# xitorch/xitorch

Hardware: AMD Instinct MI355X
Metric: eigpairs/sec of symeig(davidson) + Lanczos-role matvec GB/s (roofline.achieved), batch=64 N=16384 (higher is better)
Workload: dtype f64

## Files before the change

### xitorch_amd/csrc/xk_basis.hip

```cpp
#include "xk_common.h"

namespace xk {

template <typename T, int P>
__global__ __launch_bounds__(256) void lincomb_kernel(
    const T* __restrict__ V, const T* __restrict__ C, T* __restrict__ Out,
    int k, int N, long ldv, long sV, long sC, long sCa, long sCc, long ldo, long sO,
    T alpha, T beta, int col_tiles) {
  typedef typename Vec16<T>::type VT;
  constexpr int VN = Vec16<T>::n;
  const int b = blockIdx.x / col_tiles;
  const int ct = blockIdx.x - b * col_tiles;
  const int j = (ct * 256 + threadIdx.x) * VN;
  if (j >= N) return;
  const T* Vb = V + (long)b * sV + j;
  const T* Cb = C + (long)b * sC;
  VT acc[P];
#pragma unroll
  for (int c = 0; c < P; ++c)
#pragma unroll
    for (int v = 0; v < VN; ++v) acc[c][v] = T(0);
  int a = 0;
  for (; a + 8 <= k; a += 8) {
    VT v[8];
#pragma unroll
    for (int u = 0; u < 8; ++u) v[u] = *reinterpret_cast<const VT*>(Vb + (long)(a + u) * ldv);
#pragma unroll
    for (int c = 0; c < P; ++c) {
      T cc[8];
#pragma unroll
      for (int u = 0; u < 8; ++u) cc[u] = Cb[(long)(a + u) * sCa + c * sCc];
#pragma unroll
      for (int u = 0; u < 8; ++u)
#pragma unroll
        for (int e = 0; e < VN; ++e) acc[c][e] += cc[u] * v[u][e];
    }
  }
  for (; a + 4 <= k; a += 4) {
    VT v0 = *reinterpret_cast<const VT*>(Vb + (long)(a + 0) * ldv);
    VT v1 = *reinterpret_cast<const VT*>(Vb + (long)(a + 1) * ldv);
    VT v2 = *reinterpret_cast<const VT*>(Vb + (long)(a + 2) * ldv);
    VT v3 = *reinterpret_cast<const VT*>(Vb + (long)(a + 3) * ldv);
#pragma unroll
    for (int c = 0; c < P; ++c) {
      const T c0 = Cb[(long)(a + 0) * sCa + c * sCc], c1 = Cb[(long)(a + 1) * sCa + c * sCc];
      const T c2 = Cb[(long)(a + 2) * sCa + c * sCc], c3 = Cb[(long)(a + 3) * sCa + c * sCc];
#pragma unroll
      for (int v = 0; v < VN; ++v) {
        acc[c][v] += c0 * v0[v];
        acc[c][v] += c1 * v1[v];
        acc[c][v] += c2 * v2[v];
        acc[c][v] += c3 * v3[v];
      }
    }
  }
  for (; a < k; ++a) {
    VT v0 = *reinterpret_cast<const VT*>(Vb + (long)a * ldv);
#pragma unroll
    for (int c = 0; c < P; ++c) {
      const T c0 = Cb[(long)a * sCa + c * sCc];
#pragma unroll
      for (int v = 0; v < VN; ++v) acc[c][v] += c0 * v0[v];
    }
  }
  T* Ob = Out + (long)b * sO + j;
#pragma unroll
  for (int c = 0; c < P; ++c) {
    VT o;
    if (beta != T(0)) {
      o = *reinterpret_cast<const VT*>(Ob + (long)c * ldo);
#pragma unroll
      for (int v = 0; v < VN; ++v) o[v] = beta * o[v] + alpha * acc[c][v];
    } else {
#pragma unroll
      for (int v = 0; v < VN; ++v) o[v] = alpha * acc[c][v];
    }
    *reinterpret_cast<VT*>(Ob + (long)c * ldo) = o;
  }
}

template <typename T, int P>
__global__ __launch_bounds__(256) void ritz_residual_kernel(
    const T* __restrict__ V, const T* __restrict__ AV, const T* __restrict__ Y,
    const T* __restrict__ lam, T* __restrict__ X, T* __restrict__ Tn, T* __restrict__ rmax,
    int k, int N, long ldv, long sV, long ldav, long sAV, long sY, long sYa, long sYc, long sLam,
    long ldx, long sX, long ldt, long sT, int col_tiles) {
  typedef typename Vec16<T>::type VT;
  constexpr int VN = Vec16<T>::n;
  __shared__ T red[4];
  const int b = blockIdx.x / col_tiles;
  const int ct = blockIdx.x - b * col_tiles;
  const int j = (ct * 256 + threadIdx.x) * VN;
  const bool active = j < N;
  T local_max = T(0);
  if (active) {
    const T* Vb = V + (long)b * sV + j;
    const T* AVb = AV + (long)b * sAV + j;
    const T* Yb = Y + (long)b * sY;
    VT ax[P], xx[P];
#pragma unroll
    for (int c = 0; c < P; ++c)
#pragma unroll
      for (int v = 0; v < VN; ++v) { ax[c][v] = T(0); xx[c][v] = T(0); }
    int a = 0;
    for (; a + 4 <= k; a += 4) {
      VT v[4], w[4];
#pragma unroll
      for (int u = 0; u < 4; ++u) {
        v[u] = *reinterpret_cast<const VT*>(Vb + (long)(a + u) * ldv);
        w[u] = *reinterpret_cast<const VT*>(AVb + (long)(a + u) * ldav);
      }
#pragma unroll
      for (int c = 0; c < P; ++c) {
        T yy[4];
#pragma unroll
        for (int u = 0; u < 4; ++u) yy[u] = Yb[(long)(a + u) * sYa + c * sYc];
#pragma unroll
        for (int u = 0; u < 4; ++u)
#pragma unroll
          for (int e = 0; e < VN; ++e) {
            xx[c][e] += yy[u] * v[u][e];
            ax[c][e] += yy[u] * w[u][e];
          }
      }
    }
    for (; a + 2 <= k; a += 2) {
      VT v0 = *reinterpret_cast<const VT*>(Vb + (long)a * ldv);
      VT v1 = *reinterpret_cast<const VT*>(Vb + (long)(a + 1) * ldv);
      VT w0 = *reinterpret_cast<const VT*>(AVb + (long)a * ldav);
      VT w1 = *reinterpret_cast<const VT*>(AVb + (long)(a + 1) * ldav);
#pragma unroll
      for (int c = 0; c < P; ++c) {
        const T y0 = Yb[(long)a * sYa + c * sYc], y1 = Yb[(long)(a + 1) * sYa + c * sYc];
#pragma unroll
        for (int v = 0; v < VN; ++v) {
          xx[c][v] += y0 * v0[v];
          xx[c][v] += y1 * v1[v];
          ax[c][v] += y0 * w0[v];
          ax[c][v] += y1 * w1[v];
        }
      }
    }
    for (; a < k; ++a) {
      VT v0 = *reinterpret_cast<const VT*>(Vb + (long)a * ldv);
      VT w0 = *reinterpret_cast<const VT*>(AVb + (long)a * ldav);
#pragma unroll
      for (int c = 0; c < P; ++c) {
        const T y0 = Yb[(long)a * sYa + c * sYc];
#pragma unroll
        for (int v = 0; v < VN; ++v) { xx[c][v] += y0 * v0[v]; ax[c][v] += y0 * w0[v]; }
      }
    }
#pragma unroll
    for (int c = 0; c < P; ++c) {
      const T l = lam[(long)b * sLam + c];
      VT t;
#pragma unroll
      for (int v = 0; v < VN; ++v) {
        const T r = ax[c][v] - l * xx[c][v];
        t[v] = -r;
        T ar = r < T(0) ? -r : r;
        ar = ar != ar ? T(INFINITY) : ar;
        local_max = ar > local_max ? ar : local_max;
      }
      *reinterpret_cast<VT*>(X + (long)b * sX + (long)c * ldx + j) = xx[c];
      *reinterpret_cast<VT*>(Tn + (long)b * sT + (long)c * ldt + j) = t;
    }
  }
  local_max = wave_max(local_max);
  if ((threadIdx.x & 63) == 0) red[threadIdx.x >> 6] = local_max;
  __syncthreads();
  if (threadIdx.x == 0) {
    T m = red[0];
    m = red[1] > m ? red[1] : m;
    m = red[2] > m ? red[2] : m;
    m = red[3] > m ? red[3] : m;
    atomic_max_nonneg(rmax + b, m);
  }
}

template <typename T>
__global__ __launch_bounds__(64) void panel_chol_kernel(const T* __restrict__ G, T* __restrict__ W, int* __restrict__ info,
                                                        int B, int P, long ldg, long sG, long sW) {
  __shared__ T R[32][33];
  __shared__ T C[32][33];
  const int b = blockIdx.x;
  const int j = threadIdx.x;
  if (b >= B) return;
  const T* Gb = G + (long)b * sG;
  const bool own = j < P;
  int bad = 0;
  for (int i = 0; i < P; ++i) {
    T s = T(0);
    if (own && j >= i) {
      s = T(0.5) * (Gb[(long)i * ldg + j] + Gb[(long)j * ldg + i]);
      for (int m = 0; m < i; ++m) s -= R[m][i] * R[m][j];
      if (j == i) {
        if (!(s > T(0))) { bad = i + 1; s = T(1); }
        R[i][i] = sqrt(s);
      }
    }
    __builtin_amdgcn_fence(__ATOMIC_RELEASE, "wavefront");
    __builtin_amdgcn_wave_barrier();
    __builtin_amdgcn_fence(__ATOMIC_ACQUIRE, "wavefront");
    if (own && j > i) R[i][j] = s / R[i][i];
    if (own && j < i) R[i][j] = T(0);
    __builtin_amdgcn_fence(__ATOMIC_RELEASE, "wavefront");
    __builtin_amdgcn_wave_barrier();
    __builtin_amdgcn_fence(__ATOMIC_ACQUIRE, "wavefront");
  }
  T* Wb = W + (long)b * sW;
  if (own) {
    const int c = j;
    for (int i = P - 1; i >= 0; --i) {
      T s = (i == c) ? T(1) : T(0);
      for (int m = i + 1; m <= c; ++m) s -= R[i][m] * C[m][c];
      C[i][c] = (i <= c) ? s / R[i][i] : T(0);
    }
    for (int i = 0; i < P; ++i) Wb[(long)i * P + c] = C[i][c];
  }
  const unsigned long long flagged = __ballot(bad != 0);
  if (flagged && j == (int)(__ffsll((long long)flagged) - 1)) info[b] = bad;
}

template <typename T>
__global__ __launch_bounds__(256) void panel_transform_kernel(
    T* __restrict__ Tp, const T* __restrict__ W, int P, int N, long ldt, long sT, long sW, int col_tiles) {
  typedef typename Vec16<T>::type VT;
  constexpr int VN = Vec16<T>::n;
  const int b = blockIdx.x / col_tiles;
  const int ct = blockIdx.x - b * col_tiles;
  const int j = (ct * 256 + threadIdx.x) * VN;
  if (j >= N) return;
  T* Tb = Tp + (long)b * sT + j;
  const T* Wb = W + (long)b * sW;
  for (int c = P - 1; c >= 0; --c) {
    VT acc;
#pragma unroll
    for (int v = 0; v < VN; ++v) acc[v] = T(0);
    for (int a = 0; a <= c; ++a) {
      const T w = Wb[(long)a * P + c];
      VT t = *reinterpret_cast<const VT*>(Tb + (long)a * ldt);
#pragma unroll
      for (int v = 0; v < VN; ++v) acc[v] += w * t[v];
    }
    *reinterpret_cast<VT*>(Tb + (long)c * ldt) = acc;
  }
}

template <typename T>
static bool vec_ok(int N, long ld, long s, const void* p) {
  constexpr int VN = Vec16<T>::n;
  const long npad = ((long)N + VN - 1) / VN * VN;
  return (ld % VN == 0) && (ld >= npad || ld == 0) && (s % VN == 0) && (((uintptr_t)p & 15) == 0);
}

template <typename T>
static int lincomb(const T* V, const T* C, T* Out, int B, int k, int N, int P, long ldv, long sV,
                   long sC, long sCa, long sCc, long ldo, long sO, T alpha, T beta, hipStream_t st) {
  constexpr int VN = Vec16<T>::n;
  if (!vec_ok<T>(N, ldv, sV, V) || !vec_ok<T>(N, ldo, sO, Out)) return XK_ERR_UNSUPPORTED;
  const int ct = (N + 256 * VN - 1) / (256 * VN);
  int c0 = 0;
  while (c0 < P) {
    const int pc = (P - c0) >= 8 ? 8 : (P - c0);
    const T* Cc = C + (long)c0 * sCc;
    T* Oc = Out + (long)c0 * ldo;
    switch (pc) {
#define XK_CASE(PP)                                                                                   \
  case PP:                                                                                            \
    hipLaunchKernelGGL((lincomb_kernel<T, PP>), dim3((unsigned)((long)B * ct)), dim3(256), 0, st, V, \
                       Cc, Oc, k, N, ldv, sV, sC, sCa, sCc, ldo, sO, alpha, beta, ct);                \
    break;
      XK_CASE(1) XK_CASE(2) XK_CASE(3) XK_CASE(4) XK_CASE(5) XK_CASE(6) XK_CASE(7) XK_CASE(8)
#undef XK_CASE
    }
    XK_LAUNCH_CHECK();
    c0 += pc;
  }
  return XK_OK;
}

template <typename T>
static int ritz_residual(const T* V, const T* AV, const T* Y, const T* lam, T* X, T* Tn, T* rmax, int B,
                         int k, int N, int P, long ldv, long sV, long ldav, long sAV, long sY, long sYa,
                         long sYc, long sLam, long ldx, long sX, long ldt, long sT, hipStream_t st) {
  constexpr int VN = Vec16<T>::n;
  if (!vec_ok<T>(N, ldv, sV, V) || !vec_ok<T>(N, ldav, sAV, AV) || !vec_ok<T>(N, ldx, sX, X) ||
      !vec_ok<T>(N, ldt, sT, Tn))
    return XK_ERR_UNSUPPORTED;
  const int ct = (N + 256 * VN - 1) / (256 * VN);
  int c0 = 0;
  while (c0 < P) {
    const int pc = (P - c0) >= 8 ? 8 : (P - c0);
    switch (pc) {
#define XK_CASE(PP)                                                                                    \
  case PP:                                                                                             \
    hipLaunchKernelGGL((ritz_residual_kernel<T, PP>), dim3((unsigned)((long)B * ct)), dim3(256), 0,   \
                       st, V, AV, Y + (long)c0 * sYc, lam + c0, X + (long)c0 * ldx, Tn + (long)c0 * ldt, \
                       rmax, k, N, ldv, sV, ldav, sAV, sY, sYa, sYc, sLam, ldx, sX, ldt, sT, ct);       \
    break;
      XK_CASE(1) XK_CASE(2) XK_CASE(3) XK_CASE(4) XK_CASE(5) XK_CASE(6) XK_CASE(7) XK_CASE(8)
#undef XK_CASE
    }
    XK_LAUNCH_CHECK();
    c0 += pc;
  }
  return XK_OK;
}


template <typename T>
__global__ __launch_bounds__(256) void diag_precond_kernel(T* __restrict__ Tn, const T* __restrict__ d,
                                                            const T* __restrict__ m, const T* __restrict__ lam,
                                                            int N, int P, long ldt, long sT, long sD, long sM,
                                                            long sLam, T floor_, long total) {
  const long idx = (long)blockIdx.x * 256 + threadIdx.x;
  if (idx >= total) return;
  const long per_b = (long)P * N;
  const long b = idx / per_b;
  const long rem = idx - b * per_b;
  const int c = (int)(rem / N);
  const int n = (int)(rem - (long)c * N);
  const T mm = m ? m[b * sM + n] : T(1);
  T den = d[b * sD + n] - lam[b * sLam + c] * mm;
  if (fabs(den) < floor_) den = den < T(0) ? -floor_ : floor_;
  T* t = Tn + b * sT + (long)c * ldt + n;
  *t = *t / den;
}

template <typename T>
__global__ __launch_bounds__(64) void group_status_kernel(const T* __restrict__ rmax, const int* __restrict__ info,
                                                          const int* __restrict__ flag, T* __restrict__ orth,
                                                          double* __restrict__ status, int B) {
  const int lane = threadIdx.x;
  double m = 0.0, om_ = 0.0;
  int nan = 0, i1 = 0, i2 = 0;
  bool first = true;
  for (int b = lane; b < B; b += 64) {
    const double v = (double)rmax[b];
    nan |= (v != v);
    m = first ? v : (v > m ? v : m);
    const int a = info[b];
    i1 = first ? a : (a > i1 ? a : i1);
    if (flag) {
      const int f = flag[b];
      i2 = first ? f : (f > i2 ? f : i2);
    }
    if (orth) {
      const double ov = (double)orth[b];
      orth[b] = T(0);
      om_ = (ov != ov) ? __builtin_inf() : (ov > om_ ? ov : om_);
    }
    first = false;
  }
  double mm = first ? -__builtin_inf() : m;
  int a1 = first ? -2147483647 - 1 : i1, a2 = first ? -2147483647 - 1 : i2;
#pragma unroll
  for (int sft = 32; sft >= 1; sft >>= 1) {
    const double om = __shfl_xor(mm, sft, 64), oo = __shfl_xor(om_, sft, 64);
    const int o1 = __shfl_xor(a1, sft, 64), o2 = __shfl_xor(a2, sft, 64), on = __shfl_xor(nan, sft, 64);
    mm = om > mm ? om : mm;
    om_ = oo > om_ ? oo : om_;
    a1 = o1 > a1 ? o1 : a1;
    a2 = o2 > a2 ? o2 : a2;
    nan |= on;
  }
  if (lane == 0) {
    status[0] = nan ? __builtin_nan("") : mm;
    status[1] = (double)a1;
    status[2] = flag ? (double)a2 : 0.0;
    if (orth) status[4] = om_;
  }
// ... 76 lines not shown
```

### xitorch_amd/csrc/xk_common.h

```cpp
#pragma once
#include <hip/hip_runtime.h>
#include <stdint.h>

#define XK_WAVE 64

#define XK_OK 0
#define XK_ERR_ARG (-1)
#define XK_ERR_UNSUPPORTED (-2)

#define XK_LAUNCH_CHECK()                       \
  do {                                          \
    hipError_t e__ = hipGetLastError();         \
    if (e__ != hipSuccess) return (int)e__;     \
  } while (0)

namespace xk {

typedef double d2 __attribute__((ext_vector_type(2)));
typedef float f4 __attribute__((ext_vector_type(4)));

template <typename T> struct Vec16;
template <> struct Vec16<double> { typedef d2 type; static constexpr int n = 2; };
template <> struct Vec16<float> { typedef f4 type; static constexpr int n = 4; };

template <typename V>
__device__ __forceinline__ V ld_stream(const V* p) {
  return __builtin_nontemporal_load(p);
}

__device__ __forceinline__ double shfl_xor_t(double v, int mask) { return __shfl_xor(v, mask, 64); }
__device__ __forceinline__ float shfl_xor_t(float v, int mask) { return __shfl_xor(v, mask, 64); }

template <int CTRL, int ROW_MASK>
__device__ __forceinline__ double dpp_shift_or_zero(double v) {
  const int lo = __builtin_amdgcn_update_dpp(0, __double2loint(v), CTRL, ROW_MASK, 0xf, true);
  const int hi = __builtin_amdgcn_update_dpp(0, __double2hiint(v), CTRL, ROW_MASK, 0xf, true);
  return __hiloint2double(hi, lo);
}
template <int CTRL, int ROW_MASK>
__device__ __forceinline__ float dpp_shift_or_zero(float v) {
  return __int_as_float(__builtin_amdgcn_update_dpp(0, __float_as_int(v), CTRL, ROW_MASK, 0xf, true));
}
template <int MASK> struct PartnerCtrl;
template <> struct PartnerCtrl<8> { static constexpr int ctrl = 0x128; };
template <> struct PartnerCtrl<4> { static constexpr int ctrl = 0x141; };
template <> struct PartnerCtrl<2> { static constexpr int ctrl = 0x4e; };
template <> struct PartnerCtrl<1> { static constexpr int ctrl = 0xb1; };
template <int MASK>
__device__ __forceinline__ double lane_partner(double v) {
  const int lo = __builtin_amdgcn_update_dpp(0, __double2loint(v), PartnerCtrl<MASK>::ctrl, 0xf, 0xf, false);
  const int hi = __builtin_amdgcn_update_dpp(0, __double2hiint(v), PartnerCtrl<MASK>::ctrl, 0xf, 0xf, false);
  return __hiloint2double(hi, lo);
}
template <int MASK>
__device__ __forceinline__ float lane_partner(float v) {
  return __int_as_float(__builtin_amdgcn_update_dpp(0, __float_as_int(v), PartnerCtrl<MASK>::ctrl, 0xf, 0xf, false));
}
template <typename T>
__device__ __forceinline__ T lane_partner_rt(T v, int mask) {
  switch (mask) {
    case 8: return lane_partner<8>(v);
    case 4: return lane_partner<4>(v);
    case 2: return lane_partner<2>(v);
    case 1: return lane_partner<1>(v);
    default: return shfl_xor_t(v, mask);
  }
}
__device__ __forceinline__ double readlane63(double v) {
  const int lo = __builtin_amdgcn_readlane(__double2loint(v), 63);
  const int hi = __builtin_amdgcn_readlane(__double2hiint(v), 63);
  return __hiloint2double(hi, lo);
}
__device__ __forceinline__ float readlane63(float v) {
  return __int_as_float(__builtin_amdgcn_readlane(__float_as_int(v), 63));
}
template <typename T>
__device__ __forceinline__ T wave_sum_dpp(T v) {
  v += dpp_shift_or_zero<0x111, 0xf>(v);
  v += dpp_shift_or_zero<0x112, 0xf>(v);
  v += dpp_shift_or_zero<0x114, 0xf>(v);
  v += dpp_shift_or_zero<0x118, 0xf>(v);
  v += dpp_shift_or_zero<0x142, 0xa>(v);
  v += dpp_shift_or_zero<0x143, 0xc>(v);
  return readlane63(v);
}

template <typename T>
__device__ __forceinline__ T wave_max(T v) {
#pragma unroll
  for (int m = 32; m >= 1; m >>= 1) {
    T o = shfl_xor_t(v, m);
    v = o > v ? o : v;
  }
  return v;
}

template <int NV> struct HalvingStages {
  static constexpr int value = (NV % 2 == 0 && NV > 1) ? 1 + HalvingStages<NV / 2>::value : 0;
};
template <> struct HalvingStages<1> { static constexpr int value = 0; };
template <> struct HalvingStages<0> { static constexpr int value = 0; };

__device__ __forceinline__ double swap_add32(double a, double b) {
  auto lo = __builtin_amdgcn_permlane32_swap((unsigned)__double2loint(a), (unsigned)__double2loint(b), false, false);
  auto hi = __builtin_amdgcn_permlane32_swap((unsigned)__double2hiint(a), (unsigned)__double2hiint(b), false, false);
  return __hiloint2double((int)hi[0], (int)lo[0]) + __hiloint2double((int)hi[1], (int)lo[1]);
}
__device__ __forceinline__ float swap_add32(float a, float b) {
  auto r = __builtin_amdgcn_permlane32_swap(__float_as_uint(a), __float_as_uint(b), false, false);
  return __uint_as_float(r[0]) + __uint_as_float(r[1]);
// ... 92 lines not shown
```

### xitorch_amd/csrc/xk_symm.hip

```cpp
#include "xk_common.h"

namespace xk {

constexpr int SYMM_TRH = 1024;
constexpr long SYMM_SMALL_LAUNCH = 2200;
constexpr int SYMM_NU = 2;
constexpr int SYMM_R = 8;
constexpr long SYMM_QUEUE_ELEMS = 16;

typedef __amdgpu_buffer_rsrc_t TileRsrc;
typedef unsigned int u4 __attribute__((ext_vector_type(4)));
constexpr unsigned SYMM_OOR = 0x7ffffff0u;

#ifndef XK_SYMM_AUX
#define XK_SYMM_AUX 2
#endif
template <typename VT>
__device__ __forceinline__ VT ld_tile(const TileRsrc rsrc, unsigned lane_off, unsigned s_off) {
  const u4 raw = __builtin_amdgcn_raw_buffer_load_b128(rsrc, (int)lane_off, (int)s_off, XK_SYMM_AUX);
  return __builtin_bit_cast(VT, raw);
}

template <typename T>
__device__ __forceinline__ TileRsrc make_tile_rsrc(const T* tile_base, long bytes) {
// ... 344 lines not shown
  int j = 0;
#pragma unroll 1
  for (;;) {
#pragma unroll 1
    for (; q < NW; ++q) {
      int rb, re, c0, dg;
      if (symm_range<T, TRH, NW>(run, j, q, rb, re, c0, dg)) {
        SymmNext after = symm_next_range<T, TRH, NW>(run, j, q);
        if (after.row < 0) { after.row = run.row0; after.last = run.row0; after.col0 = N; }
        symm_rows<T, P, false>(a, tile, Xb, ldab, ldx, rb, re, run.row0, col0, N, jj, after, acc_col, xJ,
                               rowacc, lane);
      }
      __syncthreads();
    }
    T* cp = colP + (((long)b * NT + I) * P) * (long)N;
#pragma unroll
    for (int u = 0; u < NU; ++u)
      if (jj[u] < N) {
        if (flags & 1) {
#pragma unroll
          for (int c = 0; c < P; ++c) __builtin_nontemporal_store(acc_col[u][c], reinterpret_cast<VT*>(cp + (long)c * N + jj[u]));
        } else {
#pragma unroll
          for (int c = 0; c < P; ++c) *reinterpret_cast<VT*>(cp + (long)c * N + jj[u]) = acc_col[u][c];
        }
      }
    if (++j >= run.ntile) break;
    q = 0;
    col0 = (run.J0 + j) * SLAB;
    symm_tile_setup<T, P>(Xb, (int)ldx, col0, N, lanecol, jj, acc_col, xJ);
  }
  {
    const int k3 = (NW - 1) ^ run.sig;
    const int fb = run.row0 + k3 * SYMM_QR;
    int fe = fb + SYMM_QR;
    fe = fe < run.tile_end ? fe : run.tile_end;
    const int nr = fe - fb;
    T* rp = rowP + (((long)b * NSL + slot) * P) * (long)N;
    for (int idx = lane; idx < nr * P; idx += 64) {
      const int c = idx / nr, lr = idx - c * nr;
      const T v = rowacc[(fb - run.row0 + lr) * P + c];
      if (flags & 1) __builtin_nontemporal_store(v, &rp[(long)c * N + fb + lr]);
      else rp[(long)c * N + fb + lr] = v;
    }
  }
  if (!PERSIST) break;
  __syncthreads();
  item = __builtin_amdgcn_readfirstlane(s_next[par]);
  par ^= 1;
  }
}

template <typename T, int PP, bool PERS>
static int symm_launch_wide8(dim3 grid, size_t lds, hipStream_t st, const T* A, const T* Xc, T* rowP, T* colP,
                             int nruns, int N, long lda, long sA, long ldx, long sX, int NS, int NT, int NSL, int L,
                             int fl, unsigned* queue, int nitems) {
  if constexpr (sizeof(T) == 8) {
    auto kfn = dense_symm_tiles<T, PP, 2048, PERS, 8>;
    if (lds > 65536) {
      hipError_t ae = hipFuncSetAttribute(reinterpret_cast<const void*>(kfn),
                                          hipFuncAttributeMaxDynamicSharedMemorySize, (int)lds);
      if (ae != hipSuccess) return (int)ae;
    }
    hipLaunchKernelGGL(kfn, grid, dim3(512), lds, st, A, Xc, rowP, colP, nruns, N, lda, sA, ldx, sX, NS, NT, NSL, L,
                       fl, queue, nitems);
    return XK_OK;
  } else {
    return XK_ERR_UNSUPPORTED;
  }
}

static int symm_device_cus() {
  static int cus[64] = {0};
  int dev = 0;
  if (hipGetDevice(&dev) != hipSuccess || dev < 0 || dev >= 64) return 256;
  if (cus[dev] == 0) {
    int n = 0;
    if (hipDeviceGetAttribute(&n, hipDeviceAttributeMultiprocessorCount, dev) != hipSuccess || n <= 0) n = 256;
    cus[dev] = n;
  }
  return cus[dev];
}

template <typename T>
__global__ __launch_bounds__(256) void symm_fold(const T* __restrict__ rowP, const T* __restrict__ colP,
                                                  T* __restrict__ Y, int N, int P, int NS, int NT, int NSL, int L,
                                                  int slab, long ldy, long sY, long total, int flags, int trh) {
  const long idx = (long)blockIdx.x * 256 + threadIdx.x;
  if (idx >= total) return;
  const long per_b = (long)P * N;
  const long b = idx / per_b;
  const long rem = idx - b * per_b;
  const int c = (int)(rem / N);
  const int n = (int)(rem - (long)c * N);
  const int It = n / trh;
  const int jmin = (It * trh) / slab;
  const int nslot = (NS - jmin + L - 1) / L;
  T s = T(0);
  const int Imax = ((n / slab) * slab + slab - 1) / trh;
  if (flags & 2) {
    for (int r = 0; r < nslot; ++r) s += __builtin_nontemporal_load(&rowP[(((long)b * NSL + r) * P + c) * (long)N + n]);
    for (int I = 0; I <= Imax && I < NT; ++I)
      s += __builtin_nontemporal_load(&colP[(((long)b * NT + I) * P + c) * (long)N + n]);
  } else {
    for (int r = 0; r < nslot; ++r) s += rowP[(((long)b * NSL + r) * P + c) * (long)N + n];
    for (int I = 0; I <= Imax && I < NT; ++I) s += colP[(((long)b * NT + I) * P + c) * (long)N + n];
  }
  Y[b * sY + (long)c * ldy + n] = s;
}

}

extern "C" {


long xk_dense_symm_workspace_elems(int B, int N, int P, int elem_size) {
  const int vn = 16 / elem_size;
  const long slab = 256L * vn * xk::SYMM_NU;
  const long NS = (N + slab - 1) / slab, NT = (N + 511) / 512;
  const long pc = P > 6 ? 6 : P;
  return (long)B * (NS + NT) * pc * N + xk::SYMM_QUEUE_ELEMS;
}

#define XK_DEFINE_SYMM(SUF, T)                                                                              \
  static int symm_launch_##SUF(const T* A, const T* X, T* Y, T* ws, long ws_elems, int B, int N, int P,     \
                               long lda, long sA, long ldx, long sX, long ldy, long sY, int opts,           \
                               void* stream, int phase) {                                                   \
    if (B < 0 || N < 0 || P < 0 || opts < 0 || opts > 0x0fffffff) return XK_ERR_ARG;                        \
    if (B == 0 || N == 0 || P == 0) return XK_OK;                                                           \
    if (phase != 0 && P > 6) return XK_ERR_UNSUPPORTED;            \
    constexpr int VN = xk::Vec16<T>::n;                                                                     \
                       \
    const bool wide8 = sizeof(T) == 8 && (opts & 32) != 0;                                                  \
    const int NWV = wide8 ? 8 : 4;                                                                          \
    const int SLAB = NWV * 64 * VN * xk::SYMM_NU;                                                           \
    if ((N % VN) || (lda % VN) || (sA % VN) || (ldx % VN) || (sX % VN) || ((uintptr_t)A & 15) ||             \
        ((uintptr_t)X & 15) || ((uintptr_t)ws & 15))                                                        \
      return XK_ERR_UNSUPPORTED;                                                                            \
    if ((long)(wide8 ? 2048 : xk::SYMM_TRH) * lda * (long)sizeof(T) > 0x7fffffe0L) return XK_ERR_UNSUPPORTED; \
    hipStream_t st = (hipStream_t)stream;                                                                   \
    const int L = ((opts >> 8) & 0xff) ? ((opts >> 8) & 0xff) : 1, fl = 3 & ~opts;                          \
    const bool persist = (opts & 16) != 0;                                                                  \
    int nslots = (opts >> 16) & 0xfff;                                                                      \
    if (persist && nslots == 0) nslots = 2 * xk::symm_device_cus();                                         \
    if (persist && wide8) nslots = (nslots + 1) / 2;               \
    if (persist && (nslots <= 0 || ws_elems < xk::SYMM_QUEUE_ELEMS)) return XK_ERR_ARG;                     \
    unsigned* queue = persist ? reinterpret_cast<unsigned*>(ws + (ws_elems - xk::SYMM_QUEUE_ELEMS)) : nullptr; \
    if (persist) ws_elems -= xk::SYMM_QUEUE_ELEMS;                                                          \
    if (L > 64) return XK_ERR_ARG;                                                                          \
    const int NS = (N + SLAB - 1) / SLAB;                                                                   \
    const int NSL = (NS + L - 1) / L;                                                                       \
         \
    int trh = xk::SYMM_TRH;                                                                                 \
    {                                                                                                       \
      const int nt1 = (N + xk::SYMM_TRH - 1) / xk::SYMM_TRH;                                                \
      long nr1 = 0;                                                                                         \
      for (int I = 0; I < nt1; ++I) nr1 += (NS - (I * xk::SYMM_TRH) / SLAB + L - 1) / L;                    \
      if (sizeof(T) == 8 && (long)B * nr1 < xk::SYMM_SMALL_LAUNCH) trh = 512;                               \
      if (sizeof(T) == 8 && (opts & 4)) trh = 512;                                                          \
      if (opts & 8) trh = xk::SYMM_TRH;                                                                     \
      if (wide8) trh = 2048;                                                                                \
    }                                                                                                       \
    const int NT = (N + trh - 1) / trh;                                                                     \
    int nruns = 0;                                                                                          \
    for (int I = 0; I < NT; ++I) nruns += (NS - (I * trh) / SLAB + L - 1) / L;                              \
    int c0 = 0;                                                                                             \
    while (c0 < P) {                                                                                        \
      const int pc = (P - c0) >= 6 ? 6 : (P - c0);                                                          \
      const long nrow = (long)B * NSL * pc * N, ncol = (long)B * NT * pc * N;                               \
      if (ws_elems < nrow + ncol) return XK_ERR_ARG;                                                        \
      T* rowP = ws;                                                                                         \
      T* colP = ws + nrow;                                                                                  \
      const size_t lds = (size_t)trh * pc * sizeof(T);                                                      \
      const long nitems_l = (long)B * nruns;                                                                \
      if (nitems_l > 0x7fffffffL) return XK_ERR_UNSUPPORTED;                                                \
      const int nitems = (int)nitems_l;                                                                     \
      const dim3 grid((unsigned)(persist ? (nitems < nslots ? nitems : nslots) : nitems));                  \
      const T* Xc = X + (long)c0 * ldx;                                                                     \
      if (phase != 2) {                                                                                     \
        if (persist) {                                                                                      \
          hipError_t me = hipMemsetAsync(queue, 0, 64, st);                                                 \
          if (me != hipSuccess) return (int)me;                                                             \
        }                                                                                                   \
        switch (pc) {                                                                                       \
          XK_SYMM_CASE(1) XK_SYMM_CASE(2) XK_SYMM_CASE(3) XK_SYMM_CASE(4) XK_SYMM_CASE(5) XK_SYMM_CASE(6)   \
        }                                                                                                   \
        XK_LAUNCH_CHECK();                                                                                  \
      }                                                                                                     \
      if (phase != 1) {                                                                                     \
        const long total = (long)B * pc * N;                                                                \
        hipLaunchKernelGGL((xk::symm_fold<T>), dim3((unsigned)((total + 255) / 256)), dim3(256), 0, st,     \
                           rowP, colP, Y + (long)c0 * ldy, N, pc, NS, NT, NSL, L, SLAB, ldy, sY, total,     \
                           fl, trh);                                                                        \
        XK_LAUNCH_CHECK();                                                                                  \
      }                                                                                                     \
      c0 += pc;                                                                                             \
    }                                                                                                       \
    return XK_OK;                                                                                           \
  }                                                                                                         \
  int xk_dense_symm_##SUF(const T* A, const T* X, T* Y, T* ws, long ws_elems, int B, int N, int P, long lda, \
                          long sA, long ldx, long sX, long ldy, long sY, int opts, void* stream) {          \
    return symm_launch_##SUF(A, X, Y, ws, ws_elems, B, N, P, lda, sA, ldx, sX, ldy, sY, opts, stream, 0);   \
  }                                                                                                         \
  int xk_dense_symm_tiles_##SUF(const T* A, const T* X, T* ws, long ws_elems, int B, int N, int P,          \
                                long lda, long sA, long ldx, long sX, int opts, void* stream) {             \
    return symm_launch_##SUF(A, X, (T*)nullptr, ws, ws_elems, B, N, P, lda, sA, ldx, sX, 0, 0, opts,        \
                             stream, 1);                                                                    \
  }                                                                                                         \
  int xk_dense_symm_fold_##SUF(T* Y, const T* ws, long ws_elems, int B, int N, int P, long ldy, long sY,    \
                               int opts, void* stream) {                                                    \
                                         \
    return symm_launch_##SUF((const T*)ws, (const T*)ws, Y, (T*)ws, ws_elems, B, N, P, N, 0, N, 0, ldy, sY, \
                             opts, stream, 2);                                                              \
  }

#define XK_SYMM_LAUNCH(PP, RR, PERS)                                                                      \
  hipLaunchKernelGGL((xk::dense_symm_tiles<TT, PP, RR, PERS, 4>), grid, dim3(256), lds, st, A, Xc, rowP, colP, \
                     nruns, N, lda, sA, ldx, sX, NS, NT, NSL, L, fl, queue, nitems)
#define XK_SYMM_WIDE8(PP, PERS)                                                                           \
  do {                                                                                                    \
    const int wrc = xk::symm_launch_wide8<TT, PP, PERS>(grid, lds, st, A, Xc, rowP, colP, nruns, N, lda, sA, ldx, \
                                                        sX, NS, NT, NSL, L, fl, queue, nitems);           \
    if (wrc != XK_OK) return wrc;                                                                         \
  } while (0)
#define XK_SYMM_CASE(PP)                                                                                  \
  case PP:                                                                                                \
    if (wide8) {                                                                                          \
      if (persist) XK_SYMM_WIDE8(PP, true); else XK_SYMM_WIDE8(PP, false);                                \
    } else if (trh == 512) {                                                                              \
      if (persist) XK_SYMM_LAUNCH(PP, 512, true); else XK_SYMM_LAUNCH(PP, 512, false);                    \
    } else {                                                                                              \
      if (persist) XK_SYMM_LAUNCH(PP, 1024, true); else XK_SYMM_LAUNCH(PP, 1024, false);                  \
    }                                                                                                     \
    break;

#define TT double
XK_DEFINE_SYMM(f64, double)
#undef TT
#define TT float
XK_DEFINE_SYMM(f32, float)
#undef TT

}
```

### xitorch_amd/linalg/native_eig.py

```python
import os
import torch
from xitorch_amd import kernels as K
from xitorch_amd._capi import NativeLibraryError
from xitorch_amd._util import bcast_shape
from xitorch_amd.linalg._panel import PanelOperator, pad_len
from xitorch_amd.dist import allreduce_max_

__all__ = ["davidson", "exacteig", "take_eigpairs", "tallqr_extend", "native_partial_eigh"]

_PRELAUNCH = True
CHAIN_CUS = "all"
K3G_MAX_K = [1536, 1024]
K3P_MIN_K = int(os.environ.get("XITORCH_K3P_MIN_K", "80"))


def take_eigpairs(evals, evecs, neig, mode):
    if mode == "lowest":
        return evals[..., :neig], evecs[..., :neig]
    return evals[..., -neig:], evecs[..., -neig:]


def _pad(n, dtype):
    return pad_len(n)

# ... 427 lines not shown
GUARD_MAX_REDO = 3


def davidson(A, neig, mode, M=None, max_niter=1000, nguess=None, v_init="randn", max_addition=None,
             min_eps=1e-6, verbose=False, V0=None, orth_passes="auto", process_group=None, trace=None,
             rng_device="cpu", small_eigh="native", overlap="auto", precond=None, reserve_cus="auto", restart=None,
             groups="auto", chain="calls", basis_capacity=None, **unused):
    kw = dict(M=M, max_niter=max_niter, nguess=nguess, v_init=v_init, max_addition=max_addition, min_eps=min_eps,
              verbose=verbose, V0=V0, process_group=process_group, trace=trace, rng_device=rng_device,
              small_eigh=small_eigh, overlap=overlap, precond=precond, reserve_cus=reserve_cus, restart=restart,
              groups=groups, chain=chain, basis_capacity=basis_capacity, **unused)
    try:
        return _davidson(A, neig, mode, orth_passes=orth_passes, **kw)
    except _GuardFailure as err:
        if isinstance(orth_passes, int) and orth_passes >= 3:
            raise RuntimeError("xitorch_amd davidson: %s" % err)
        first = dict(trace) if trace is not None else None
        try:
            res = _davidson(A, neig, mode, orth_passes=3, **kw)
        except _GuardFailure as err2:
            raise RuntimeError("xitorch_amd davidson: %s (also with three orthogonalisation passes)" % err2)
        if trace is not None:
            trace["orth_rerun"] = {"reason": str(err), "first_run": {k: first.get(k) for k in ("niter", "orth_redo")}}
        return res


class _GuardPolicy:

    def __init__(self, dtype, k_start):
        self.good, self.bad = GUARD_GOOD[dtype], GUARD_BAD[dtype]
        self.k_good = k_start
        self.history, self.redo = [], []
        self._restarts = 0

    def seen(self, guard, nrestart):
        self.history.append(guard)
        if nrestart != self._restarts:
            self._restarts, self.k_good = nrestart, None

    def void(self, chol_flag, guard):
        return chol_flag != 0 or guard > self.bad

    def roll_back(self, chol_flag, guard, k_rr, niter, trace):
        if self.k_good is None or self.k_good >= k_rr or len(self.redo) >= GUARD_MAX_REDO:
            if chol_flag != 0 and not self.redo:
                raise RuntimeError("xitorch_amd davidson: the panel Gram matrix is not positive definite "
                                   "(linearly dependent guess/residual vectors)")
            if trace is not None:
                trace.update(niter=niter, orth_redo=self.redo, orth_guard_history=self.history)
            raise _GuardFailure("the Ritz block lost its orthonormality (max|X^T M X - I| = %.2e at iteration %d, "
                                "basis of %d vectors) and no earlier basis is left to return to" % (guard, niter, k_rr))
        self.redo.append({"iter": niter, "guard": guard, "chol_flag": chol_flag, "k_from": k_rr, "k_to": self.k_good,
                          "passes": 2 + len(self.redo)})
        return self.k_good, 2 + len(self.redo) - 1

    def passed(self, guard, k_rr):
        if guard <= self.good:
            self.k_good = k_rr
            return True
        return False


class _Plan:
    __slots__ = ("two", "ngrp", "reserve_cus", "spans", "ops", "streams", "k1_streams", "k1_sched", "distributed")


def _plan_groups(A, whole, M, B, N, p, dtype, device, precond, overlap, groups, reserve_cus, k1_streams_opt,
                 reserve_schedule, process_group):
    plan = _Plan()
    nA = 1
    for d in A.shape[:-2]:
        nA *= d
    can_two = M is None and whole.kind == "dense" and not whole.flip and nA == B and B >= 2 \
        and not (precond is not None and not isinstance(precond, (str, torch.Tensor)))
    big = B * N * N * (8 if dtype == torch.float64 else 4) >= 2 ** 33
    two = can_two and (overlap is True or (overlap == "auto" and big))
    ngrp = 2
    if two:
        if groups == "auto":
            ngrp = 2
        else:
            ngrp = max(2, min(int(groups), B))
    reserve_auto = reserve_cus == "auto"
    if reserve_cus == "auto":
        wide_symm = whole.kind == "dense" and whole.symm and dtype == torch.float32 and \
            K.SYMM_WIDE_MIN_P <= p <= K.SYMM_WIDE_MAX_P and N >= K.SYMM_WIDE_MIN_N and N % 64 == 0
        reserve_cus = 32 if wide_symm else 64
        if can_two and K.K1S_OPTS is None and whole.kind == "dense" and whole.symm and whole.symm_narrow and p <= 6 \
                and (k1_streams_opt == "auto" or bool(k1_streams_opt)):
            total_cus = torch.cuda.get_device_properties(device).multi_processor_count
            if K.k1s_auto_opts(B // ngrp, N, dtype, max(1, total_cus - 32), pipelined=True) & K.K1S_PERSIST:
                reserve_cus = 32
    grp_streams, k1_streams, k1_sched = None, [None], None
    if two:
        try:
            chain_reserved = CHAIN_CUS == "reserved" or (CHAIN_CUS == "auto" and wide_symm and bool(K.K1SW_OPTS & 8))
            if chain_reserved and reserve_cus > 0:
                grp_streams = [K.masked_stream(device, reserve_cus, slot=1 + g, only_reserved=True) for g in range(ngrp)]
            else:
                grp_streams = [K.masked_stream(device, 0, slot=1 + g) for g in range(ngrp)]
            k1_stream = K.masked_stream(device, reserve_cus)
            k1_streams = [k1_stream] * ngrp
            if k1_streams_opt == "auto":
                k1o = K.K1S_OPTS if K.K1S_OPTS is not None else \
                    K.k1s_auto_opts(B // ngrp, N, dtype, K.stream_cus(k1_stream), pipelined=True)
                split_k1 = bool(k1o & K.K1S_PERSIST) and whole.kind == "dense" and whole.symm \
                    and whole.symm_narrow and p <= 6
            else:
                split_k1 = bool(k1_streams_opt)
            if k1_streams_opt == "auto" and not split_k1 and whole.kind == "dense" and whole.symm and \
                    dtype == torch.float32 and K.SYMM_WIDE_MIN_P <= p <= K.SYMM_WIDE_MAX_P and \
                    N >= K.SYMM_WIDE_MIN_N and N % 64 == 0:
                split_k1 = bool(K._k1sw_opts(k1_stream, B // ngrp, N, pipelined=True) & K.K1SW_PERSIST)
            if split_k1:
                k1_streams = [K.masked_stream(device, reserve_cus, slot=64 + g) for g in range(ngrp)]
                sched = reserve_schedule
                if sched == "auto":
                    sched = [(0, 32), (132, 64)] if (reserve_auto and reserve_cus == 32) else None
                if sched:
                    k1_sched = [(int(kf), [K.masked_stream(device, int(reserve_cus if cu is None else cu), slot=64 + g)
                                           for g in range(ngrp)]) for (kf, cu) in sched]
        except NativeLibraryError as err:
            import warnings
            warnings.warn("xitorch_amd davidson: CU-masked streams unavailable (%s); running one batch group" % err)
            two = False
    distributed = process_group is not None and torch.distributed.get_world_size(process_group) > 1
    if distributed:
        g_local = ngrp if two else 1
        g_all = torch.tensor([-float(g_local)], dtype=torch.float64, device=device)
        torch.distributed.all_reduce(g_all, op=torch.distributed.ReduceOp.MAX, group=process_group)
        g_common = int(round(-g_all.item()))
        if g_common < g_local:
            if g_common <= 1:
                two = False
            else:
                ngrp = g_common
                grp_streams, k1_streams = grp_streams[:ngrp], k1_streams[:ngrp]
                k1_sched = [(kf, sts[:ngrp]) for (kf, sts) in k1_sched] if k1_sched is not None else None
    if two:
        cuts = [(B * g) // ngrp for g in range(ngrp + 1)]
        spans = [(cuts[g], cuts[g + 1]) for g in range(ngrp)]
        ops = [_PanelOperator(_sub_operator(A, B, N, b0, b1), [b1 - b0], b1 - b0, N) for (b0, b1) in spans]
        cur = torch.cuda.current_stream()
        streams = grp_streams
        for st in streams + list(set(k1_streams)) + [t for (_, sts) in (k1_sched or []) for t in sts]:
            st.wait_stream(cur)
    else:
        spans, ops, streams, k1_streams, k1_sched = [(0, B)], [whole], [torch.cuda.current_stream()], [None], None
    plan.two, plan.ngrp, plan.reserve_cus, plan.spans, plan.ops, plan.streams = two, ngrp, reserve_cus, spans, ops, streams
    plan.k1_streams, plan.k1_sched, plan.distributed = k1_streams, k1_sched, distributed
    return plan


def _preconditioner(precond, whole, M, bdims, B, N, dtype, device):
    if precond is None:
        return None
    from xitorch_amd.linop import LinearOperator as _LinOp
    if isinstance(precond, str):
        if precond.lower() not in ("diag", "jacobi", "davidson"):
            raise RuntimeError("Unknown davidson preconditioner: %s" % precond)
        dA = whole.diagonal()
        dM = _PanelOperator(M, bdims, B, N).diagonal() if M is not None else None
        return ("diag", dA, dM)
    if isinstance(precond, torch.Tensor):
        if precond.shape[-1] != N:
            raise RuntimeError("precond diagonal must have shape (*batch, %d), got %s" % (N, tuple(precond.shape)))
        dA = precond.to(device=device, dtype=dtype).expand(*bdims, N).reshape(B, N).contiguous()
        dM = _PanelOperator(M, bdims, B, N).diagonal() if M is not None else None
        return ("diag", dA, dM)
# ... 317 lines not shown
```

Measured before the change: 1827.

## Use buffer-resource ring-buffered row loads in lincomb, ritz residual and symm fold

Rewrites the basis lincomb and Ritz-residual kernels to keep a register ring of in-flight row loads (depth 16 and 8), issued as raw buffer loads with scalar offsets and guarded out-of-range so the memory pipeline stays full. symm_fold is vectorized to 16-byte accesses per thread with the same ring prefetch. A Python fix hoists wide_symm out of the auto branch so it is defined when reserve_cus is explicit. This aims to hide memory latency in bandwidth-bound streaming kernels, at the cost of higher register pressure and new span limits that fall back to unsupported for large strides.

```diff
diff --git a/xitorch_amd/csrc/xk_basis.hip b/xitorch_amd/csrc/xk_basis.hip
--- a/xitorch_amd/csrc/xk_basis.hip
+++ b/xitorch_amd/csrc/xk_basis.hip
@@ -1,6 +1,12 @@
 #include "xk_common.h"
 
 namespace xk {
+
+constexpr int LINCOMB_RING = 16;
+constexpr int RITZ_RING = 8;
+#ifndef XK_BASIS_AUX
+#define XK_BASIS_AUX 0
+#endif
 
 template <typename T, int P>
 __global__ __launch_bounds__(256) void lincomb_kernel(
@@ -9,58 +15,56 @@
     T alpha, T beta, int col_tiles) {
   typedef typename Vec16<T>::type VT;
   constexpr int VN = Vec16<T>::n;
+  constexpr int D = LINCOMB_RING;
   const int b = blockIdx.x / col_tiles;
   const int ct = blockIdx.x - b * col_tiles;
   const int j = (ct * 256 + threadIdx.x) * VN;
   if (j >= N) return;
-  const T* Vb = V + (long)b * sV + j;
+  const T* Vb = V + (long)b * sV;
   const T* Cb = C + (long)b * sC;
+  const unsigned loff = (unsigned)j * (unsigned)sizeof(T);
+  const unsigned ldvb = (unsigned)(ldv * (long)sizeof(T));
   VT acc[P];
 #pragma unroll
   for (int c = 0; c < P; ++c)
 #pragma unroll
     for (int v = 0; v < VN; ++v) acc[c][v] = T(0);
+  VT ring[D];
+  RowRsrc rs = make_row_rsrc(Vb);
+#pragma unroll
+  for (int u = 0; u < D; ++u) ring[u] = ld_row<VT, XK_BASIS_AUX>(rs, u < k ? loff : ROW_OOR, (unsigned)u * ldvb);
   int a = 0;
-  for (; a + 8 <= k; a += 8) {
-    VT v[8];
-#pragma unroll
-    for (int u = 0; u < 8; ++u) v[u] = *reinterpret_cast<const VT*>(Vb + (long)(a + u) * ldv);
-#pragma unroll
-    for (int c = 0; c < P; ++c) {
-      T cc[8];
-#pragma unroll
-      for (int u = 0; u < 8; ++u) cc[u] = Cb[(long)(a + u) * sCa + c * sCc];
-#pragma unroll
-      for (int u = 0; u < 8; ++u)
-#pragma unroll
-        for (int e = 0; e < VN; ++e) acc[c][e] += cc[u] * v[u][e];
-    }
-  }
-  for (; a + 4 <= k; a += 4) {
-    VT v0 = *reinterpret_cast<const VT*>(Vb + (long)(a + 0) * ldv);
-    VT v1 = *reinterpret_cast<const VT*>(Vb + (long)(a + 1) * ldv);
-    VT v2 = *reinterpret_cast<const VT*>(Vb + (long)(a + 2) * ldv);
-    VT v3 = *reinterpret_cast<const VT*>(Vb + (long)(a + 3) * ldv);
-#pragma unroll
-    for (int c = 0; c < P; ++c) {
-      const T c0 = Cb[(long)(a + 0) * sCa + c * sCc], c1 = Cb[(long)(a + 1) * sCa + c * sCc];
-      const T c2 = Cb[(long)(a + 2) * sCa + c * sCc], c3 = Cb[(long)(a + 3) * sCa + c * sCc];
-#pragma unroll
-      for (int v = 0; v < VN; ++v) {
-        acc[c][v] += c0 * v0[v];
-        acc[c][v] += c1 * v1[v];
-        acc[c][v] += c2 * v2[v];
-        acc[c][v] += c3 * v3[v];
-      }
-    }
-  }
-  for (; a < k; ++a) {
-    VT v0 = *reinterpret_cast<const VT*>(Vb + (long)a * ldv);
-#pragma unroll
-    for (int c = 0; c < P; ++c) {
-      const T c0 = Cb[(long)a * sCa + c * sCc];
-#pragma unroll
-      for (int v = 0; v < VN; ++v) acc[c][v] += c0 * v0[v];
+  for (; a + D <= k; a += D) {
+#pragma unroll
+    for (int h = 0; h < D; h += 4) {
+      T cc[4][P];
+#pragma unroll
+      for (int u = 0; u < 4; ++u)
+#pragma unroll
+        for (int c = 0; c < P; ++c) cc[u][c] = Cb[(long)(a + h + u) * sCa + c * sCc];
+#pragma unroll
+      for (int u = 0; u < 4; ++u) {
+        const VT v = ring[h + u];
+#pragma unroll
+        for (int c = 0; c < P; ++c)
+#pragma unroll
+          for (int e = 0; e < VN; ++e) acc[c][e] += cc[u][c] * v[e];
+        ring[h + u] = ld_row<VT, XK_BASIS_AUX>(rs, a + D + h + u < k ? loff : ROW_OOR, (unsigned)(D + h + u) * ldvb);
+        __builtin_amdgcn_sched_barrier(0);
+      }
+    }
+    rs = make_row_rsrc(Vb + (long)(a + D) * ldv);
+  }
+#pragma unroll
+  for (int u = 0; u < D - 1; ++u) {
+    if (a + u < k) {
+      const VT v = ring[u];
+#pragma unroll
+      for (int c = 0; c < P; ++c) {
+        const T c0 = Cb[(long)(a + u) * sCa + c * sCc];
+#pragma unroll
+        for (int e = 0; e < VN; ++e) acc[c][e] += c0 * v[e];
+      }
     }
   }
   T* Ob = Out + (long)b * sO + j;
@@ -87,6 +91,7 @@
     long ldx, long sX, long ldt, long sT, int col_tiles) {
   typedef typename Vec16<T>::type VT;
   constexpr int VN = Vec16<T>::n;
+  constexpr int D = RITZ_RING;
   __shared__ T red[4];
   const int b = blockIdx.x / col_tiles;
   const int ct = blockIdx.x - b * col_tiles;
@@ -94,61 +99,61 @@
   const bool active = j < N;
   T local_max = T(0);
   if (active) {
-    const T* Vb = V + (long)b * sV + j;
-    const T* AVb = AV + (long)b * sAV + j;
+    const T* Vb = V + (long)b * sV;
+    const T* AVb = AV + (long)b * sAV;
     const T* Yb = Y + (long)b * sY;
+    const unsigned loff = (unsigned)j * (unsigned)sizeof(T);
+    const unsigned ldvb = (unsigned)(ldv * (long)sizeof(T)), ldavb = (unsigned)(ldav * (long)sizeof(T));
     VT ax[P], xx[P];
 #pragma unroll
     for (int c = 0; c < P; ++c)
 #pragma unroll
       for (int v = 0; v < VN; ++v) { ax[c][v] = T(0); xx[c][v] = T(0); }
+    VT rv[D], rw[D];
+    RowRsrc dv = make_row_rsrc(Vb), dw = make_row_rsrc(AVb);
+#pragma unroll
+    for (int u = 0; u < D; ++u) {
+      rv[u] = ld_row<VT, XK_BASIS_AUX>(dv, u < k ? loff : ROW_OOR, (unsigned)u * ldvb);
+      rw[u] = ld_row<VT, XK_BASIS_AUX>(dw, u < k ? loff : ROW_OOR, (unsigned)u * ldavb);
+    }
     int a = 0;
-    for (; a + 4 <= k; a += 4) {
-      VT v[4], w[4];
-#pragma unroll
-      for (int u = 0; u < 4; ++u) {
-        v[u] = *reinterpret_cast<const VT*>(Vb + (long)(a + u) * ldv);
-        w[u] = *reinterpret_cast<const VT*>(AVb + (long)(a + u) * ldav);
-      }
-#pragma unroll
-      for (int c = 0; c < P; ++c) {
-        T yy[4];
-#pragma unroll
-        for (int u = 0; u < 4; ++u) yy[u] = Yb[(long)(a + u) * sYa + c * sYc];
+    for (; a + D <= k; a += D) {
+#pragma unroll
+      for (int h = 0; h < D; h += 4) {
+        T yy[4][P];
 #pragma unroll
         for (int u = 0; u < 4; ++u)
 #pragma unroll
-          for (int e = 0; e < VN; ++e) {
-            xx[c][e] += yy[u] * v[u][e];
-            ax[c][e] += yy[u] * w[u][e];
-          }
-      }
-    }
-    for (; a + 2 <= k; a += 2) {
-      VT v0 = *reinterpret_cast<const VT*>(Vb + (long)a * ldv);
-      VT v1 = *reinterpret_cast<const VT*>(Vb + (long)(a + 1) * ldv);
-      VT w0 = *reinterpret_cast<const VT*>(AVb + (long)a * ldav);
-      VT w1 = *reinterpret_cast<const VT*>(AVb + (long)(a + 1) * ldav);
-#pragma unroll
-      for (int c = 0; c < P; ++c) {
-        const T y0 = Yb[(long)a * sYa + c * sYc], y1 = Yb[(long)(a + 1) * sYa + c * sYc];
-#pragma unroll
-        for (int v = 0; v < VN; ++v) {
-          xx[c][v] += y0 * v0[v];
-          xx[c][v] += y1 * v1[v];
-          ax[c][v] += y0 * w0[v];
-          ax[c][v] += y1 * w1[v];
+          for (int c = 0; c < P; ++c) yy[u][c] = Yb[(long)(a + h + u) * sYa + c * sYc];
+#pragma unroll
+        for (int u = 0; u < 4; ++u) {
+          const VT v = rv[h + u], w = rw[h + u];
+#pragma unroll
+          for (int c = 0; c < P; ++c)
+#pragma unroll
+            for (int e = 0; e < VN; ++e) {
+              xx[c][e] += yy[u][c] * v[e];
+              ax[c][e] += yy[u][c] * w[e];
+            }
+          const unsigned off = a + D + h + u < k ? loff : ROW_OOR;
+          rv[h + u] = ld_row<VT, XK_BASIS_AUX>(dv, off, (unsigned)(D + h + u) * ldvb);
+          rw[h + u] = ld_row<VT, XK_BASIS_AUX>(dw, off, (unsigned)(D + h + u) * ldavb);
+          __builtin_amdgcn_sched_barrier(0);
         }
       }
-    }
-    for (; a < k; ++a) {
-      VT v0 = *reinterpret_cast<const VT*>(Vb + (long)a * ldv);
-      VT w0 = *reinterpret_cast<const VT*>(AVb + (long)a * ldav);
-#pragma unroll
-      for (int c = 0; c < P; ++c) {
-        const T y0 = Yb[(long)a * sYa + c * sYc];
-#pragma unroll
-        for (int v = 0; v < VN; ++v) { xx[c][v] += y0 * v0[v]; ax[c][v] += y0 * w0[v]; }
+      dv = make_row_rsrc(Vb + (long)(a + D) * ldv);
+      dw = make_row_rsrc(AVb + (long)(a + D) * ldav);
+    }
+#pragma unroll
+    for (int u = 0; u < D - 1; ++u) {
+      if (a + u < k) {
+        const VT v = rv[u], w = rw[u];
+#pragma unroll
+        for (int c = 0; c < P; ++c) {
+          const T y0 = Yb[(long)(a + u) * sYa + c * sYc];
+#pragma unroll
+          for (int e = 0; e < VN; ++e) { xx[c][e] += y0 * v[e]; ax[c][e] += y0 * w[e]; }
+        }
       }
     }
 #pragma unroll
@@ -256,10 +261,16 @@
 }
 
 template <typename T>
+static bool ring_ok(int N, long ld, int depth) {
+  return ld >= 0 && (2L * depth * ld + N + 16) * (long)sizeof(T) <= ROW_SPAN_MAX;
+}
+
+template <typename T>
 static int lincomb(const T* V, const T* C, T* Out, int B, int k, int N, int P, long ldv, long sV,
                    long sC, long sCa, long sCc, long ldo, long sO, T alpha, T beta, hipStream_t st) {
   constexpr int VN = Vec16<T>::n;
   if (!vec_ok<T>(N, ldv, sV, V) || !vec_ok<T>(N, ldo, sO, Out)) return XK_ERR_UNSUPPORTED;
+  if (!ring_ok<T>(N, ldv, LINCOMB_RING)) return XK_ERR_UNSUPPORTED;
   const int ct = (N + 256 * VN - 1) / (256 * VN);
   int c0 = 0;
   while (c0 < P) {
@@ -289,6 +300,7 @@
   if (!vec_ok<T>(N, ldv, sV, V) || !vec_ok<T>(N, ldav, sAV, AV) || !vec_ok<T>(N, ldx, sX, X) ||
       !vec_ok<T>(N, ldt, sT, Tn))
     return XK_ERR_UNSUPPORTED;
+  if (!ring_ok<T>(N, ldv, RITZ_RING) || !ring_ok<T>(N, ldav, RITZ_RING)) return XK_ERR_UNSUPPORTED;
   const int ct = (N + 256 * VN - 1) / (256 * VN);
   int c0 = 0;
   while (c0 < P) {
diff --git a/xitorch_amd/csrc/xk_common.h b/xitorch_amd/csrc/xk_common.h
--- a/xitorch_amd/csrc/xk_common.h
+++ b/xitorch_amd/csrc/xk_common.h
@@ -26,6 +26,25 @@
 template <typename V>
 __device__ __forceinline__ V ld_stream(const V* p) {
   return __builtin_nontemporal_load(p);
+}
+
+typedef __amdgpu_buffer_rsrc_t RowRsrc;
+constexpr unsigned ROW_OOR = 0x7ffffff0u;
+constexpr long ROW_SPAN_MAX = 0x7fffffe0L;
+
+template <typename T>
+__device__ __forceinline__ RowRsrc make_row_rsrc(const T* base) {
+  const uint64_t v = reinterpret_cast<uint64_t>(base);
+  const uint32_t lo = __builtin_amdgcn_readfirstlane((uint32_t)v);
+  const uint32_t hi = __builtin_amdgcn_readfirstlane((uint32_t)(v >> 32));
+  void* p = reinterpret_cast<void*>(((uint64_t)hi << 32) | lo);
+  return __builtin_amdgcn_make_buffer_rsrc(p, (short)0, (int)ROW_SPAN_MAX, 0x00020000);
+}
+template <typename VT, int AUX>
+__device__ __forceinline__ VT ld_row(const RowRsrc rsrc, unsigned lane_off, unsigned s_off) {
+  typedef unsigned int u4_ __attribute__((ext_vector_type(4)));
+  const u4_ raw = __builtin_amdgcn_raw_buffer_load_b128(rsrc, (int)lane_off, (int)s_off, AUX);
+  return __builtin_bit_cast(VT, raw);
 }
 
 __device__ __forceinline__ double shfl_xor_t(double v, int mask) { return __shfl_xor(v, mask, 64); }
diff --git a/xitorch_amd/csrc/xk_symm.hip b/xitorch_amd/csrc/xk_symm.hip
--- a/xitorch_amd/csrc/xk_symm.hip
+++ b/xitorch_amd/csrc/xk_symm.hip
@@ -450,31 +450,59 @@
   return cus[dev];
 }
 
-template <typename T>
+constexpr int SYMM_FOLD_RING = 8;
+template <typename T, int AUX>
 __global__ __launch_bounds__(256) void symm_fold(const T* __restrict__ rowP, const T* __restrict__ colP,
                                                   T* __restrict__ Y, int N, int P, int NS, int NT, int NSL, int L,
-                                                  int slab, long ldy, long sY, long total, int flags, int trh) {
-  const long idx = (long)blockIdx.x * 256 + threadIdx.x;
-  if (idx >= total) return;
-  const long per_b = (long)P * N;
-  const long b = idx / per_b;
-  const long rem = idx - b * per_b;
-  const int c = (int)(rem / N);
-  const int n = (int)(rem - (long)c * N);
-  const int It = n / trh;
+                                                  int slab, long ldy, long sY, int col_tiles, int yvec, int trh) {
+  typedef typename Vec16<T>::type VT;
+  constexpr int VN = Vec16<T>::n;
+  constexpr int D = SYMM_FOLD_RING;
+  const int ct = blockIdx.x % col_tiles;
+  const int bc = blockIdx.x / col_tiles;
+  const int b = bc / P, c = bc - b * P;
+  const int n0 = ct * 256 * VN;
+  const int n = n0 + (int)threadIdx.x * VN;
+  const int It = n0 / trh;
   const int jmin = (It * trh) / slab;
   const int nslot = (NS - jmin + L - 1) / L;
-  T s = T(0);
-  const int Imax = ((n / slab) * slab + slab - 1) / trh;
-  if (flags & 2) {
-    for (int r = 0; r < nslot; ++r) s += __builtin_nontemporal_load(&rowP[(((long)b * NSL + r) * P + c) * (long)N + n]);
-    for (int I = 0; I <= Imax && I < NT; ++I)
-      s += __builtin_nontemporal_load(&colP[(((long)b * NT + I) * P + c) * (long)N + n]);
+  int ncol = ((n0 / slab) * slab + slab - 1) / trh + 1;
+  ncol = ncol < NT ? ncol : NT;
+  const int nl = nslot + ncol;
+  const unsigned loff = n < N ? (unsigned)n * (unsigned)sizeof(T) : ROW_OOR;
+  const unsigned step = (unsigned)((long)P * N * (long)sizeof(T));
+  const RowRsrc rrow = make_row_rsrc(rowP + ((long)b * NSL * P + c) * (long)N);
+  const RowRsrc rcol = make_row_rsrc(colP + ((long)b * NT * P + c) * (long)N);
+  VT ring[D];
+#pragma unroll
+  for (int u = 0; u < D; ++u) {
+    const bool row = u < nslot;
+    ring[u] = ld_row<VT, AUX>(row ? rrow : rcol, u < nl ? loff : ROW_OOR, (unsigned)(row ? u : u - nslot) * step);
+  }
+  VT s;
+#pragma unroll
+  for (int e = 0; e < VN; ++e) s[e] = T(0);
+  for (int i0 = 0; i0 < nl; i0 += D) {
+#pragma unroll
+    for (int u = 0; u < D; ++u) {
+      if (i0 + u < nl) {
+#pragma unroll
+        for (int e = 0; e < VN; ++e) s[e] += ring[u][e];
+      }
+      const int i = i0 + D + u;
+      const bool row = i < nslot;
+      ring[u] = ld_row<VT, AUX>(row ? rrow : rcol, i < nl ? loff : ROW_OOR, (unsigned)(row ? i : i - nslot) * step);
+      __builtin_amdgcn_sched_barrier(0);
+    }
+  }
+  if (n >= N) return;
+  T* y = Y + b * sY + (long)c * ldy + n;
+  if (yvec) {
+    *reinterpret_cast<VT*>(y) = s;
   } else {
-    for (int r = 0; r < nslot; ++r) s += rowP[(((long)b * NSL + r) * P + c) * (long)N + n];
-    for (int I = 0; I <= Imax && I < NT; ++I) s += colP[(((long)b * NT + I) * P + c) * (long)N + n];
-  }
-  Y[b * sY + (long)c * ldy + n] = s;
+#pragma unroll
+    for (int e = 0; e < VN; ++e) y[e] = s[e];
+  }
 }
 
 }
@@ -556,10 +584,19 @@
         XK_LAUNCH_CHECK();                                                                                  \
       }                                                                                                     \
       if (phase != 1) {                                                                                     \
-        const long total = (long)B * pc * N;                                                                \
-        hipLaunchKernelGGL((xk::symm_fold<T>), dim3((unsigned)((total + 255) / 256)), dim3(256), 0, st,     \
-                           rowP, colP, Y + (long)c0 * ldy, N, pc, NS, NT, NSL, L, SLAB, ldy, sY, total,     \
-                           fl, trh);                                                                        \
+        const int fct = (N + 256 * VN - 1) / (256 * VN);                                                    \
+        const long fblk = (long)B * pc * fct;                                                               \
+                  \
+        if (fblk > 0x7fffffffL || ((long)(NSL > NT ? NSL : NT) * pc + 1) * N * (long)sizeof(T) > xk::ROW_SPAN_MAX) \
+          return XK_ERR_UNSUPPORTED;                                                                        \
+        T* Yc = Y + (long)c0 * ldy;                                                                         \
+        const int yvec = !(ldy % VN) && !(sY % VN) && !((uintptr_t)Yc & 15);                                \
+        if (fl & 2)                                                                                         \
+          hipLaunchKernelGGL((xk::symm_fold<T, 2>), dim3((unsigned)fblk), dim3(256), 0, st, rowP, colP, Yc, N, pc, \
+                             NS, NT, NSL, L, SLAB, ldy, sY, fct, yvec, trh);                                \
+        else                                                                                                \
+          hipLaunchKernelGGL((xk::symm_fold<T, 0>), dim3((unsigned)fblk), dim3(256), 0, st, rowP, colP, Yc, N, pc, \
+                             NS, NT, NSL, L, SLAB, ldy, sY, fct, yvec, trh);                                \
         XK_LAUNCH_CHECK();                                                                                  \
       }                                                                                                     \
       c0 += pc;                                                                                             \
diff --git a/xitorch_amd/linalg/native_eig.py b/xitorch_amd/linalg/native_eig.py
--- a/xitorch_amd/linalg/native_eig.py
+++ b/xitorch_amd/linalg/native_eig.py
@@ -533,9 +533,9 @@
         else:
             ngrp = max(2, min(int(groups), B))
     reserve_auto = reserve_cus == "auto"
+    wide_symm = whole.kind == "dense" and whole.symm and dtype == torch.float32 and \
+        K.SYMM_WIDE_MIN_P <= p <= K.SYMM_WIDE_MAX_P and N >= K.SYMM_WIDE_MIN_N and N % 64 == 0
     if reserve_cus == "auto":
-        wide_symm = whole.kind == "dense" and whole.symm and dtype == torch.float32 and \
-            K.SYMM_WIDE_MIN_P <= p <= K.SYMM_WIDE_MAX_P and N >= K.SYMM_WIDE_MIN_N and N % 64 == 0
         reserve_cus = 32 if wide_symm else 64
         if can_two and K.K1S_OPTS is None and whole.kind == "dense" and whole.symm and whole.symm_narrow and p <= 6 \
                 and (k1_streams_opt == "auto" or bool(k1_streams_opt)):
```

New measurement: 1814. No clear change (-0.8%).
